# wenzhang-dev/bitcaskDB

Measured on AMD Instinct MI355X. Metric: WAL record decode+CRC GiB/s (device-resident), 4 KiB values, 1/2/4/8 MI355X, higher is better.
Workload: dtype u8; 1 GPU; config B: 1073743514 B WAL segment per GPU, NsSize 20, 100 B keys, 4 KiB values, device-resident decode+CRC+record parse; seg_bytes=1073743514, records=253846, fragments=286402, parallelism=one independent segment per GPU x1

## Files before the change

bitcaskdb_amd/csrc/bcw_decode.hip:

```cpp
#include <hip/hip_runtime.h>

#include <cstdint>

#include "bcw_internal.h"
#include "bcw_parse.h"

namespace bcw {

enum { M_FIRST_BAD = 0,
       M_NE = 1,
       M_NFRAGS = 4, M_DONE_CRC = 5,
       M_T_CRC0 = 10, M_T_FIN = 11,
       M_ABORT = 12,
       M_BAD_CRC = 14,
       M_BAD_TYPE = 15 };

__device__ __forceinline__ uint32_t rotl32(uint32_t x, int r) { return (x << r) | (x >> (32 - r)); }

__device__ __forceinline__ void read_header(const uint8_t* __restrict__ seg, uint64_t seg_len, uint64_t off,
                                            uint32_t& crc, uint32_t& len, uint32_t& type) {
  const uint64_t a = off & ~3ull;
  uint32_t w0, w1, w2;
  if (a + 12 <= seg_len) {
    const uint32_t* q = reinterpret_cast<const uint32_t*>(seg + a);
// ... 412 lines not shown
    const uint64_t be = wg * 64 + 64 < nblocks ? wg * 64 + 64 : nblocks;
    fbase[be] = (uint32_t)(total < 0xffffffffull ? total : 0xffffffffull);
    rbase[be] = (uint32_t)(total_e < 0xffffffffull ? total_e : 0xffffffffull);
    if (wg == nwg - 1) {
      misc[M_NFRAGS] = total;
      misc[M_NE] = total_e;
    }
  }
}

__device__ __forceinline__ uint32_t xor3(uint32_t a, uint32_t b, uint32_t c) {
  return __builtin_amdgcn_bitop3_b32(a, b, c, 0x96);
}
__device__ __forceinline__ uint32_t apply_fwd(const uint32_t* __restrict__ fwd, uint32_t lane, uint32_t x) {
  const uint8_t* b = reinterpret_cast<const uint8_t*>(fwd);
  const uint32_t lane4 = 4u * lane;
  auto at = [&](int i) -> uint32_t {
    const uint32_t sh = 4 * i >= 8 ? (x >> (4 * i - 8)) : (x << (8 - 4 * i));
    return *reinterpret_cast<const uint32_t*>(b + (((sh & 0xf00u) | lane4) + 4096u * (uint32_t)i));
  };
  const uint32_t r0 = at(0), r1 = at(1), r2 = at(2), r3 = at(3), r4 = at(4), r5 = at(5), r6 = at(6), r7 = at(7);
  return xor3(xor3(r0, r1, r2), xor3(r3, r4, r5), r6) ^ r7;
}
__device__ __forceinline__ uint32_t apply_op(const uint32_t* __restrict__ c, uint32_t x) {
  uint32_t r = 0;
#pragma unroll
  for (int i = 0; i < 8; ++i) r ^= c[i * 16 + ((x >> (4 * i)) & 15u)];
  return r;
}

__device__ __forceinline__ uint4 load16_slow(const uint8_t* __restrict__ seg, uint64_t seg_len, int64_t o) {
  uint64_t lo = 0, hi = 0;
#pragma unroll 1
  for (int i = 0; i < 16; ++i) {
    const int64_t q = o + i;
    const uint64_t byte = (q >= 0 && (uint64_t)q < seg_len) ? seg[q] : 0u;
    if (i < 8) lo |= byte << (8 * i); else hi |= byte << (8 * (i - 8));
  }
  return make_uint4((uint32_t)lo, (uint32_t)(lo >> 32), (uint32_t)hi, (uint32_t)(hi >> 32));
}
__device__ __forceinline__ uint4 load16_safe(const uint8_t* __restrict__ seg, uint64_t seg_len, int64_t o) {
  if (o >= 0 && (uint64_t)o + 16 <= seg_len) return *reinterpret_cast<const uint4*>(seg + o);
  return load16_slow(seg, seg_len, o);
}


template <int N>
__device__ __forceinline__ uint32_t reg_byte(const uint32_t (&h)[N], uint32_t pos) {
  uint32_t t[N];
#pragma unroll
  for (int i = 0; i < N; ++i) t[i] = h[i];
  const uint32_t wi = pos >> 2;
  int n = N;
#pragma unroll
  for (int bit = 0; bit < 6; ++bit) {
    if (n <= 1) break;
    const bool hi = (wi >> bit) & 1u;
#pragma unroll
    for (int i = 0; i < (N + 1) / 2; ++i) {
      if (i < (n + 1) / 2) t[i] = (2 * i + 1 < n) ? (hi ? t[2 * i + 1] : t[2 * i]) : t[2 * i];
    }
    n = (n + 1) / 2;
  }
  return (t[0] >> (8u * (pos & 3u))) & 0xffu;
}

constexpr int kHeadWords = 16;
constexpr int kTailWords = 8;

__device__ __attribute__((noinline)) uint32_t walk_byte(const uint8_t* __restrict__ seg, const Frag* __restrict__ frags,
                                                        uint32_t start_off, uint32_t f_first, uint32_t f_last,
                                                        uint64_t pos) {
  uint64_t beg = 0;
  for (uint32_t cf = f_first;; ++cf) {
    const Frag f = frags[cf];
    if (pos < beg + f.len || cf >= f_last)
      return seg[(uint64_t)start_off + (uint64_t)f.blk * kBlock + f.start + (pos - beg)];
    beg += f.len;
  }
}

struct RegReader {
  uint32_t h[kHeadWords];
  uint32_t t[kTailWords];
  uint32_t nhead;
  uint64_t tstart;
  uint64_t tend;
  const uint8_t* seg;
  const Frag* frags;
  uint32_t start_off;
  uint32_t f_first, f_last;
  __device__ __forceinline__ uint32_t operator()(uint64_t pos) {
    if (pos < nhead) return reg_byte(h, (uint32_t)pos);
    if (pos >= tstart && pos < tend) return reg_byte(t, (uint32_t)(pos - tstart));
    return walk_byte(seg, frags, start_off, f_first, f_last, pos);
  }
};

template <int N>
__device__ __forceinline__ void load_words(const uint8_t* __restrict__ seg, uint64_t seg_len, uint64_t base,
                                           uint32_t (&w)[N]) {
  if (base + 4u * N <= seg_len) {
#pragma unroll
    for (int k = 0; k < N / 4; ++k) {
      uint4 v;
      __builtin_memcpy(&v, seg + base + 16 * k, 16);
      w[4 * k + 0] = v.x; w[4 * k + 1] = v.y; w[4 * k + 2] = v.z; w[4 * k + 3] = v.w;
    }
  } else {
#pragma unroll
    for (int k = 0; k < N / 4; ++k) {
      const uint4 v = load16_safe(seg, seg_len, (int64_t)(base + 16 * k));
      w[4 * k + 0] = v.x; w[4 * k + 1] = v.y; w[4 * k + 2] = v.z; w[4 * k + 3] = v.w;
    }
  }
}

struct EmitArgs {
  const uint8_t* seg;
  uint64_t seg_len;
  bcw_decode_params p;
  const Frag* frags;
  const uint32_t* fbase;
  const uint32_t* rbase;
  const uint2* bsum;
  bcw_record_table tab;
  uint64_t* misc;
  uint32_t kb_flags;
  uint64_t* kb_stamps;
};


struct EmitState {
  uint64_t acc;
  int64_t nzb;
  uint32_t nzk, nzs;
  uint64_t rec;
};
__device__ __forceinline__ uint2 emit_prefetch(const EmitArgs& A, uint64_t b0, uint32_t lane) {
  return b0 > lane ? A.bsum[b0 - 1 - lane] : make_uint2(0xffff0000u, kSumHasE);
}

__device__ __forceinline__ EmitState emit_state(const EmitArgs& A, uint64_t b0, uint32_t lane, uint2 s, uint32_t rec) {
  EmitState st{0, -1, 0, 0, rec};
  uint64_t acc = 0;
  for (uint64_t top = b0; top > 0;) {
    if (top != b0) {
      const uint64_t q = top - 1 - lane;
      s = top > lane ? A.bsum[q] : make_uint2(0xffff0000u, kSumHasE);
    }
    const uint64_t he = __ballot((s.y & kSumHasE) != 0u);
    const uint32_t stop = he ? (uint32_t)__builtin_ctzll(he) : 63u;
    const bool contrib = lane <= stop;
    uint32_t ta = contrib ? (s.x & 0xffffu) : 0u;
#pragma unroll
    for (int d = 32; d >= 1; d >>= 1) ta += (uint32_t)__shfl_xor((int)ta, d, 64);
    acc += (uint32_t)__builtin_amdgcn_readfirstlane(ta);
    const uint64_t nzm = __ballot(contrib && (s.x >> 16) != 0xffffu);
    if (nzm) {
      const uint32_t L = 63u - __builtin_clzll(nzm);
      st.nzb = (int64_t)(top - 1 - L);
      st.nzk = (uint32_t)__builtin_amdgcn_readlane((int)(s.x >> 16), L);
      st.nzs = (uint32_t)__builtin_amdgcn_readlane((int)(s.y & 0xffffu), L);
    }
    if (he) break;
    top = top > 64 ? top - 64 : 0;
  }
  st.acc = acc;
  return st;
}

template <bool NOSTORE = false, bool NOPARSE = false, typename Hook>
__device__ __forceinline__ void emit_chunks(const EmitArgs& A, const EmitState& es, uint64_t f0, uint64_t f1,
                                            uint32_t lane, Hook&& hook) {
  if (f0 >= f1) {
    hook();
    return;
  }
  const Frag* __restrict__ frags = A.frags;
  const uint32_t start_off = A.p.start_off;
  uint64_t acc = es.acc, off = 0;
  uint32_t first = 0;
  if (es.nzb >= 0) {
    off = (uint64_t)start_off + (uint64_t)es.nzb * kBlock + es.nzs;
    first = A.fbase[es.nzb] + es.nzk;
  }
  uint64_t rec = es.rec;
  const bool hint = A.p.mode == BCW_MODE_HINT;
  for (uint64_t c0 = f0; c0 < f1; c0 += 64) {
    const uint64_t g = c0 + lane;
    const bool valid = g < f1;
    const uint4 fr = reinterpret_cast<const uint4*>(frags)[valid ? g : f1 - 1];
    if (c0 == f0) hook();
    Frag f;
    __builtin_memcpy(&f, &fr, sizeof f);
    if (!valid) f = Frag{};
    const uint32_t len = valid ? f.len : 0u;
    const uint64_t D = (uint64_t)start_off + (uint64_t)f.blk * kBlock + f.start;
    const bool isE = valid && (f.type == BCW_RECORD_FULL || f.type == BCW_RECORD_LAST);
    const uint64_t E = __ballot(isE);
    const uint64_t NZ = __ballot(valid && len > 0);
    const uint32_t S = wave_add_scan(len, lane);
    const uint64_t below = (lane == 0) ? 0ull : (~0ull >> (64 - lane));
    const uint64_t pm = E & below;
    const int prev = pm ? 63 - __builtin_clzll(pm) : -1;
    const uint32_t S_prev = __shfl(S, prev < 0 ? 0 : prev, 64);
    const uint64_t between = (uint64_t)(S - len) - (prev < 0 ? 0u : S_prev);
    const uint64_t acc_before = (prev < 0 ? acc : 0ull) + between;
    const uint64_t range = prev < 0 ? below : (below & ~(~0ull >> (63 - prev)));
    const uint64_t nzr = NZ & range;
    const int fnz = nzr ? __builtin_ctzll(nzr) : 0;
    const uint64_t D_fnz = __shfl(D, fnz, 64);
    const uint64_t V = __ballot(valid);
    const int last_valid = V ? 63 - __builtin_clzll(V) : -1;
    const uint32_t S_tot = __shfl(S, last_valid < 0 ? 0 : last_valid, 64);
    const int lastE = E ? 63 - __builtin_clzll(E) : -1;
    uint64_t acc2, off2;
    uint32_t first2;
    {
      const uint32_t S_lastE = __shfl(S, lastE < 0 ? 0 : lastE, 64);
      const uint64_t after = lastE < 0 ? V : (V & ~(~0ull >> (63 - lastE)));
      const uint64_t nza = NZ & after;
      const int fa = nza ? __builtin_ctzll(nza) : 0;
      const uint64_t D_fa = __shfl(D, fa, 64);
      if (lastE >= 0) {
        acc2 = (uint64_t)(S_tot - S_lastE);
        off2 = D_fa;
        first2 = (uint32_t)(c0 + fa);
      } else {
        acc2 = acc + S_tot;
        if (acc > 0 || !nza) { off2 = off; first2 = first; }
        else { off2 = D_fa; first2 = (uint32_t)(c0 + fa); }
      }
    }
    uint64_t foff;
    uint32_t ffrag;
    if (acc_before == 0) { foff = D; ffrag = (uint32_t)g; }
    else if (prev < 0 && acc > 0) { foff = off; ffrag = first; }
    else { foff = D_fnz; ffrag = (uint32_t)(c0 + fnz); }
    const bool full = f.type == BCW_RECORD_FULL;
    const uint32_t src = full ? (uint32_t)g : ffrag;
    const bool src_here = src >= c0 && src < c0 + 64;
    const uint32_t sw0 = (uint32_t)__shfl((int)f.blk, src_here ? (int)(src - c0) : (int)lane, 64);
    const uint32_t sw1 = (uint32_t)__shfl((int)((uint32_t)f.start | ((uint32_t)f.len << 16)),
                                          src_here ? (int)(src - c0) : (int)lane, 64);
    const bool nx_here = src + 1u >= c0 && src + 1u < c0 + 64;
    const uint32_t sx0 = (uint32_t)__shfl((int)f.blk, nx_here ? (int)(src + 1u - c0) : (int)lane, 64);
    const uint32_t sx1 = (uint32_t)__shfl((int)((uint32_t)f.start | ((uint32_t)f.len << 16)),
                                          nx_here ? (int)(src + 1u - c0) : (int)lane, 64);
    if (isE) {
      const uint64_t size = full ? (uint64_t)len : acc_before + len;
      const uint64_t r = rec + __builtin_popcountll(E & below);
      Frag fs = f;
      if (!full) {
        if (src_here) { fs.blk = sw0; fs.start = (uint16_t)sw1; fs.len = (uint16_t)(sw1 >> 16); }
        else fs = frags[src];
      }
      RegReader rd;
      const uint64_t a0 = (uint64_t)start_off + (uint64_t)fs.blk * kBlock + fs.start;
      uint64_t want = size < 64u ? size : 64u;
      if (want > fs.len) want = fs.len;
      rd.nhead = (uint32_t)want;
      load_words(A.seg, A.seg_len, a0, rd.h);
      rd.tstart = rd.tend = ~0ull;
      if (hint) {
        uint64_t nt = size < 32u ? size : 32u;
        if (nt > len) nt = len;
        rd.tstart = size - nt;
        load_words(A.seg, A.seg_len, D + len - nt, rd.t);
      } else if (want < (size < 64u ? size : 64u)) {
        Frag f2;
        if (nx_here) { f2.blk = sx0; f2.start = (uint16_t)sx1; f2.len = (uint16_t)(sx1 >> 16); }
        else f2 = frags[src + 1u];
        load_words(A.seg, A.seg_len, (uint64_t)start_off + (uint64_t)f2.blk * kBlock + f2.start, rd.t);
        uint64_t n2 = f2.len < 32u ? f2.len : 32u;
        if (n2 > size - want) n2 = size - want;
        rd.tstart = want;
        rd.tend = want + n2;
      } else {
#pragma unroll
        for (int k = 0; k < kTailWords; ++k) rd.t[k] = 0;
      }
      rd.seg = A.seg; rd.frags = frags; rd.start_off = start_off;
      rd.f_first = src; rd.f_last = (uint32_t)g;
      uint8_t status, hdr, flags, etag_off;
      uint64_t key_len, val_len, meta_len, expire, aux0, aux1;
      if (NOPARSE) {
        status = 0; hdr = (uint8_t)rd.h[0]; flags = (uint8_t)rd.h[5]; etag_off = 0;
        key_len = rd.h[6] ^ rd.h[9]; val_len = rd.h[7] ^ rd.h[12]; meta_len = rd.h[8] ^ rd.h[15]; expire = rd.h[10];
        aux0 = rd.t[0]; aux1 = rd.t[1];
      } else {
        parse_record(A.p, rd, size, status, hdr, flags, etag_off, key_len, val_len, meta_len, expire, aux0, aux1);
      }
      const bcw_record_table& tab = A.tab;
      if (NOSTORE) {
        if (status == 0xeeu) tab.foff[r] = foff ^ size ^ expire ^ aux0 ^ aux1 ^ key_len ^ val_len ^ meta_len ^ hdr ^ flags ^ etag_off;
      } else if (r < tab.capacity) {
        tab.foff[r] = foff;
        tab.size[r] = size;
        tab.expire[r] = expire;
        if (tab.aux0) tab.aux0[r] = aux0;
        if (tab.aux1) tab.aux1[r] = aux1;
        tab.key_len[r] = (uint32_t)key_len;
        tab.val_len[r] = (uint32_t)val_len;
        tab.meta_len[r] = (uint32_t)meta_len;
        tab.first_frag[r] = src;
        tab.emit_frag[r] = (uint32_t)g;
        tab.hdr_size[r] = hdr;
        tab.flags[r] = flags;
        tab.etag_off[r] = etag_off;
        tab.status[r] = status;
      }
      if (status != BCW_ST_OK) atomicMin((unsigned long long*)&A.misc[M_FIRST_BAD], (unsigned long long)r);
    }
    rec += __builtin_popcountll(E);
    acc = acc2;
    off = off2;
    first = first2;
  }
}

struct ItemMeta {
  uint64_t bb;
  uint2 s;
  uint32_t f0, f1, rec;
};
__device__ __forceinline__ uint32_t ld_const(const uint32_t* p, uint64_t i) {
  return ((const __attribute__((address_space(4))) uint32_t*)p)[i];
}
__device__ __forceinline__ ItemMeta item_meta(const EmitArgs& A, uint64_t it, uint64_t bpw, uint64_t cb0, uint64_t cb1,
                                              uint32_t lane) {
  ItemMeta m;
  m.bb = cb0 + it * bpw < cb1 ? cb0 + it * bpw : cb1 - 1;
  const uint64_t be = m.bb + bpw < cb1 ? m.bb + bpw : cb1;
  m.s = emit_prefetch(A, m.bb, lane);
  m.f0 = ld_const(A.fbase, m.bb);
  m.f1 = ld_const(A.fbase, be);
  m.rec = ld_const(A.rbase, m.bb);
  return m;
}

__device__ __forceinline__ void finalize(const EmitArgs& A, uint64_t nblocks, uint64_t frag_cap, uint32_t tail_panic, uint64_t gen,
                         bcw_decode_result* __restrict__ res, uint32_t lane) {
  uint64_t* misc = A.misc;
  const uint64_t bad_crc = __hip_atomic_load(&misc[M_BAD_CRC], __ATOMIC_RELAXED, __HIP_MEMORY_SCOPE_AGENT);
  const uint64_t bad_type = __hip_atomic_load(&misc[M_BAD_TYPE], __ATOMIC_RELAXED, __HIP_MEMORY_SCOPE_AGENT);
  const uint64_t fb = __hip_atomic_load(&misc[M_FIRST_BAD], __ATOMIC_RELAXED, __HIP_MEMORY_SCOPE_AGENT);
  const uint64_t nfr = __hip_atomic_load(&misc[M_NFRAGS], __ATOMIC_RELAXED, __HIP_MEMORY_SCOPE_AGENT);
  const uint64_t abort_site = __hip_atomic_load(&misc[M_ABORT], __ATOMIC_RELAXED, __HIP_MEMORY_SCOPE_AGENT);
  const uint64_t err = bad_crc < bad_type ? bad_crc : bad_type;
  uint64_t lim = err < frag_cap ? err : frag_cap;
  uint64_t nrec = __hip_atomic_load(&misc[M_NE], __ATOMIC_RELAXED, __HIP_MEMORY_SCOPE_AGENT);
  if (lim < nfr && abort_site == 0ull) {
    uint64_t lo = 0, hi = nblocks;
    while (hi - lo > 1) {
      const uint64_t step = (hi - lo + 63) / 64;
      const uint64_t q = lo + (uint64_t)lane * step;
      const bool le = q < hi && A.fbase[q] <= lim;
      const uint64_t m = __ballot(le);
      const uint32_t L = m ? 63u - __builtin_clzll(m) : 0u;
      lo = lo + (uint64_t)L * step;
      hi = lo + step < hi ? lo + step : hi;
    }
    uint64_t cnt = 0;
    for (uint64_t c0 = A.fbase[lo]; c0 < lim; c0 += 64) {
      const uint64_t g = c0 + lane;
      const uint32_t ty = g < lim ? A.frags[g].type : 0u;
      cnt += (uint64_t)__builtin_popcountll(__ballot(ty == BCW_RECORD_FULL || ty == BCW_RECORD_LAST));
    }
    nrec = (uint64_t)A.rbase[lo] + cnt;
  }
  if (lane != 0) return;
  bcw_decode_result r{};
  r.n_records = nrec;
  r.n_records_total = nrec;
  r.err_frag = err;
  r.err_class = err == ~0ull ? BCW_ERR_NONE : (bad_crc <= bad_type ? BCW_ERR_CRC : BCW_ERR_TYPE);
  r.n_frags = err != ~0ull ? err + 1 : nfr;
  if (r.err_class == BCW_ERR_NONE && tail_panic) r.err_class = BCW_ERR_PANIC;
  if (abort_site != 0ull) {
    r.err_class = BCW_ERR_INTERNAL;
    r.err_frag = abort_site;
    r.n_records = r.n_records_total = 0;
    nrec = 0;
  }
  r.err_file_off = 0;
  if (err != ~0ull && err < frag_cap && abort_site == 0ull) {
    const Frag f = A.frags[err];
    r.err_file_off = (uint64_t)A.p.start_off + (uint64_t)f.blk * kBlock + f.start - kHdr;
  }
  r.first_bad_record = fb < nrec ? (int32_t)(fb < 0x7fffffffull ? fb : 0x7fffffffull) : -1;
  r.n_blocks = nblocks;
  r.retry_frag_capacity = (nfr > frag_cap && abort_site == 0ull) ? nfr : 0;
  r.generation = gen;
  *res = r;
  if (abort_site != 0ull) misc[M_NFRAGS] = 0;
  misc[M_DONE_CRC] = 0;
  misc[M_BAD_CRC] = ~0ull;
  misc[M_FIRST_BAD] = ~0ull;
  misc[M_BAD_TYPE] = ~0ull;
  misc[M_ABORT] = 0;
}

struct StreamFrag {
  int64_t gs, ge;
  uint32_t J;
};

struct SliceLane2 {
  uint32_t base;
  uint32_t sel[4];
};
__device__ __forceinline__ SliceLane2 slice_lane2(uint32_t lane) {
  SliceLane2 s;
  const uint32_t g = (lane >> 3) & 3u, copy = lane & 7u;
  s.base = 0;
#pragma unroll
  for (uint32_t k = 0; k < 4; ++k) {
    const uint32_t slot = (k + g) & 3u;
    s.base |= (slot * 32u + copy * 4u) << (8u * k);
    s.sel[k] = 0x0c0c0000u | ((4u + slot) << 8) | k;
  }
  return s;
}
template <bool SH>
__device__ __forceinline__ uint32_t slice4_step2(const uint8_t* __restrict__ tb, const SliceLane2& sl, uint32_t x,
                                                 uint32_t next) {
  constexpr uint32_t o = SH ? 128u : 0u;
  const uint32_t a0 = *reinterpret_cast<const uint32_t*>(tb + __builtin_amdgcn_perm(x, sl.base, sl.sel[0]) + o);
  const uint32_t a1 = *reinterpret_cast<const uint32_t*>(tb + __builtin_amdgcn_perm(x, sl.base, sl.sel[1]) + o);
  const uint32_t a2 = *reinterpret_cast<const uint32_t*>(tb + __builtin_amdgcn_perm(x, sl.base, sl.sel[2]) + o);
  const uint32_t a3 = *reinterpret_cast<const uint32_t*>(tb + __builtin_amdgcn_perm(x, sl.base, sl.sel[3]) + o);
  return xor3(xor3(a0, a1, a2), a3, next);
}
template <bool CAP>
__device__ __forceinline__ uint32_t chain_piece2(const uint8_t* __restrict__ tb, const SliceLane2& sl, uint32_t seed,
                                                 const uint32_t (&w)[kSPW], uint32_t K = 0, uint32_t* cap = nullptr) {
  uint32_t x = seed ^ w[0];
  uint32_t st[kSPW - 1];
#pragma unroll
  for (int q = 0; q < kSPW - 1; ++q) {
    x = slice4_step2<false>(tb, sl, x, w[q + 1]);
    if (CAP) st[q] = x ^ w[q + 1];
  }
  if (CAP) *cap = K == 1u ? st[0] : (K == 2u ? st[1] : st[2]);
  return slice4_step2<true>(tb, sl, x, 0u);
}

__device__ __forceinline__ uint64_t c_safe_bound(uint64_t seg_len) { return (seg_len + 4u + kSChunk - 1u) / kSChunk; }

__device__ __forceinline__ uint4 lds_entry(const uint32_t* __restrict__ tab, uint32_t idx) {
  return *reinterpret_cast<const uint4*>(tab + 4u * idx);
}
__device__ __forceinline__ void mask_gap(uint32_t (&x)[kSPW], const uint32_t (&w)[kSPW], int32_t pb, uint32_t J,
                                         uint32_t lane, const uint32_t* __restrict__ lds) {
  const uint32_t g = min((uint32_t)(pb - (int32_t)(kSPiece * lane) + 6), (uint32_t)(kS2GapN - 1));
  const uint4 S = lds_entry(lds + kS2Gap, g);
  x[0] = __builtin_amdgcn_perm(J, w[0], S.x);
  x[1] = __builtin_amdgcn_perm(J, w[1], S.y);
  x[2] = __builtin_amdgcn_perm(J, w[2], S.z);
  x[3] = __builtin_amdgcn_perm(J, w[3], S.w);
}
__device__ __forceinline__ void mask_chunk(uint32_t (&x)[kSPW], const uint32_t (&w)[kSPW], int32_t pa, int32_t pb,
                                           int32_t pc, uint32_t J, uint32_t lane, const uint32_t* __restrict__ lds) {
  const int32_t q = (int32_t)(kSPiece * lane);
  const uint4 A = lds_entry(lds + kS2Ge, (uint32_t)min(max(pa - q, 0), kS2GeN - 1));
// ... 177 lines not shown
};
__device__ __forceinline__ XBalIn xbal_load(const XBal* __restrict__ xb, uint32_t lane) {
  const uint32_t y = lane & 7u;
  XBalIn v;
  v.t = __hip_atomic_load(&xb->t[y], __ATOMIC_RELAXED, __HIP_MEMORY_SCOPE_AGENT);
  v.n = __hip_atomic_load(&xb->n[y], __ATOMIC_RELAXED, __HIP_MEMORY_SCOPE_AGENT);
  v.w = xb->w[y];
  v.on = xb->on;
  return v;
}
__device__ __forceinline__ void xbal_update(XBal* __restrict__ xb, uint32_t lane, const XBalIn& in) {
  const uint32_t y = lane & 7u;
  const uint64_t t = in.t, n = in.n;
  const float Ty = n && t ? (float)t / (float)n : 0.0f;
  const bool all = __ballot(lane < 8u && Ty > 0.0f) == 0xffull && in.on != 0u;
  float sT = lane < 8u ? Ty : 0.0f;
#pragma unroll
  for (int d = 32; d >= 1; d >>= 1) sT += __shfl_xor(sT, d, 64);
  if (lane < 8u) {
    if (all) {
      const float wy = (float)in.w * (1.0f + 0.5f * ((sT / 8.0f) / Ty - 1.0f));
      const float d = fminf(fmaxf(rintf((wy - 65536.0f) / 256.0f), -51.0f), 64.0f);
      xb->w[y] = (uint32_t)(65536 + 256 * (int32_t)d);
    }
    xb->t[y] = 0;
    xb->n[y] = 0;
  }
}

template <int ABL = 0>
__global__ __launch_bounds__(kCrcThreads) void k_crc(const uint8_t* __restrict__ seg, uint64_t seg_len,
                                                     uint32_t start_off, uint64_t nblocks,
                                                     const uint32_t* __restrict__ fbase, uint8_t* __restrict__ fok,
                                                     const uint4* __restrict__ srec,
                                                     uint64_t frag_cap, Tables tabs, EmitArgs ea,
                                                     uint32_t tail_panic, uint64_t gen,
                                                     bcw_decode_result* __restrict__ res,
                                                     uint64_t* __restrict__ misc, uint64_t cb0, uint64_t cb1,
                                                     uint32_t nwg_total, const uint32_t* __restrict__ wstart,
                                                     XBal* __restrict__ xb) {
  __shared__ __attribute__((aligned(16))) uint32_t lds[kS2Image];
  __shared__ CrcTail s_tail;
  __shared__ uint32_t s_wdone;
  __shared__ uint32_t s_eq;
  __shared__ __attribute__((aligned(16))) uint32_t s_rem[kCrcWaves];
  __shared__ uint32_t s_sdone;
  __shared__ unsigned long long s_tsum;
  __shared__ uint64_t s_t0;
  const uint32_t tid = threadIdx.x;
  const uint32_t lane = tid & 63u;
  const uint32_t wave = __builtin_amdgcn_readfirstlane(tid >> 6);
  if (tid < (uint32_t)kCrcWaves) s_rem[tid] = 0;
  if (ea.kb_stamps && lane == 0) {
    uint64_t* q = ea.kb_stamps + 8 * ((uint64_t)blockIdx.x * kCrcWaves + wave);
    q[4] = wall_clock64();
    q[5] = __builtin_amdgcn_s_memtime();
    q[7] = ((uint64_t)__builtin_amdgcn_s_getreg(20 | (31 << 11)) << 32) | __builtin_amdgcn_s_getreg(4 | (31 << 11));
  }
  if (tid == 0) {
    s_wdone = 0;
    s_eq = 0;
    s_sdone = 0;
    s_tsum = 0;
    s_t0 = wall_clock64();
    s_tail = CrcTail{ea, res, misc, nblocks, frag_cap, gen, cb0, cb1, tail_panic, nwg_total};
  }
  {
    const uint4* src4 = reinterpret_cast<const uint4*>(tabs.lds_image2);
    uint4* dst4 = reinterpret_cast<uint4*>(lds);
    constexpr uint32_t kLop4 = kS2SliceOff / 4, kKop4 = kS2KopOff / 4, kEnd4 = kS2Image / 4;
    constexpr uint32_t kN4 = kLop4 + (kEnd4 - kKop4);
    constexpr int kPer = (int)((kN4 + kCrcThreads - 1) / kCrcThreads);
    static_assert(kS2Slice == 256 * 64 && kCrcThreads * 2 == 256 * 8, "slice rows: 256 x 8 distinct dwords");
    auto at = [](uint32_t i) { return i < kLop4 ? i : i - kLop4 + kKop4; };
    uint4 v[kPer];
#pragma unroll
    for (int k2 = 0; k2 < kPer; ++k2) {
      const uint32_t i = tid + k2 * kCrcThreads;
      v[k2] = i < kN4 ? src4[at(i)] : make_uint4(0, 0, 0, 0);
    }
    const uint32_t* src1 = tabs.lds_image2 + kS2SliceOff;
    uint32_t sv[2];
#pragma unroll
    for (int k2 = 0; k2 < 2; ++k2) {
      const uint32_t t = tid + k2 * kCrcThreads;
      sv[k2] = src1[(t >> 3) * 64u + (t & 7u) * 8u];
    }
#pragma unroll
    for (int k2 = 0; k2 < kPer; ++k2) {
      const uint32_t i = tid + k2 * kCrcThreads;
      if (i < kN4) dst4[at(i)] = v[k2];
    }
#pragma unroll
    for (int k2 = 0; k2 < 2; ++k2) {
      const uint32_t t = tid + k2 * kCrcThreads;
      uint4* d = reinterpret_cast<uint4*>(lds + kS2SliceOff + (t >> 3) * 64u + (t & 7u) * 8u);
      d[0] = make_uint4(sv[k2], sv[k2], sv[k2], sv[k2]);
      d[1] = make_uint4(sv[k2], sv[k2], sv[k2], sv[k2]);
    }
  }
  __syncthreads();
  const uint64_t gw = (uint64_t)blockIdx.x * kCrcWaves + wave;
  const uint64_t f0 = wstart[gw];
  uint64_t f1 = wstart[gw + 1];
  if (f1 > frag_cap) f1 = frag_cap;
  if (f0 > f1) f1 = f0;
  const bool aborted = __builtin_amdgcn_readfirstlane(
                           (uint32_t)__hip_atomic_load(&misc[M_ABORT], __ATOMIC_RELAXED, __HIP_MEMORY_SCOPE_AGENT)) != 0u;
  if (aborted) f1 = f0;
  if (blockIdx.x == 0 && tid == 0) misc[M_T_CRC0] = wall_clock64();
  const uint32_t nfr = f1 > f0 ? (uint32_t)(f1 - f0) : 0u;
  uint64_t n_items = 0;
  auto emit_items = [&](uint64_t max_items) {
    asm volatile("" ::: "memory");
    CrcTail T;
    {
      static_assert(sizeof(CrcTail) % 4 == 0, "CrcTail words");
      const uint32_t* src = reinterpret_cast<const uint32_t*>(&s_tail);
      uint32_t* dst = reinterpret_cast<uint32_t*>(&T);
#pragma unroll
      for (int k = 0; k < (int)(sizeof(CrcTail) / 4); ++k) dst[k] = __builtin_amdgcn_readfirstlane(src[k]);
    }
    const EmitArgs& A = T.ea;
    if ((ABL & 8) || (A.kb_flags & 1u) ||
        __builtin_amdgcn_readfirstlane(
            (uint32_t)__hip_atomic_load(&T.misc[M_ABORT], __ATOMIC_RELAXED, __HIP_MEMORY_SCOPE_AGENT)) != 0u)
      return;
    const uint64_t cb0t = T.cb0, cb1t = T.cb1, fcap = T.frag_cap;
    const uint32_t cnt = (uint32_t)(cb1t - cb0t), G = gridDim.x, wg = blockIdx.x;
    const uint64_t fc0 = A.fbase[cb0t], fc1 = A.fbase[cb1t];
    const uint32_t nf_all = (uint32_t)(fc1 > fc0 ? (fc1 - fc0 < fcap ? fc1 - fc0 : fcap) : 0);
    uint32_t bpw = nf_all ? (64u * cnt) / nf_all : cnt;
    if (bpw < 1u) bpw = 1u;
    bpw = __builtin_amdgcn_readfirstlane(bpw);
    const uint32_t cq = cnt / G, cr = cnt % G;
    const uint32_t B0 = cq * wg + (cr * wg) / G, B1 = cq * (wg + 1u) + (cr * (wg + 1u)) / G;
    const uint64_t i0 = __builtin_amdgcn_readfirstlane((B0 + bpw - 1u) / bpw),
                   nitems = __builtin_amdgcn_readfirstlane((B1 + bpw - 1u) / bpw);
    auto deq = [&]() -> uint64_t {
      uint32_t j = 0;
      if (lane == 0) j = atomicAdd(&s_eq, 1u);
      j = __builtin_amdgcn_readfirstlane(j);
      return i0 + j;
    };
    uint64_t taken = 0;
    uint64_t it = deq();
    ItemMeta m = item_meta(A, it, bpw, cb0t, cb1t, lane);
    while (it < nitems) {
      ++taken;
      const EmitState es = emit_state(A, m.bb, lane, m.s, m.rec);
      const uint64_t mf1 = m.f1 < fcap ? m.f1 : fcap;
      uint64_t nx = ~0ull;
      ItemMeta mn = m;
      emit_chunks<(ABL & 4096) != 0, (ABL & 131072) != 0>(A, es, m.f0, mf1, lane, [&]() {
        if (taken < max_items) {
          nx = deq();
          mn = item_meta(A, nx, bpw, cb0t, cb1t, lane);
        }
      });
      it = nx;
      m = mn;
    }
    n_items += taken;
  };
  if (ABL & 64) emit_items(~0ull);
  if (ABL & 16384) {
    for (uint32_t q = 0; q < 4u; ++q) {
      const uint32_t a = nfr * q / 4u, b = nfr * (q + 1u) / 4u;
      stream_verify<(ABL & 8388608) != 0>(seg, seg_len, fok, srec, f0 + a, b - a, lds, lane, misc, s_rem,
                                          (wave & 3u) * 4u + (wave >> 2),
                                          reinterpret_cast<const uint8_t*>(tabs.lds_image2));
    }
  } else if (!(ABL & 32768))
    stream_verify<(ABL & 8388608) != 0>(seg, seg_len, fok, srec, f0, nfr, lds, lane, misc, s_rem,
                                        (wave & 3u) * 4u + (wave >> 2),
                                        reinterpret_cast<const uint8_t*>(tabs.lds_image2));
  __builtin_amdgcn_s_setprio(0);
  if (lane == 0) {
    atomicAdd(&s_tsum, (unsigned long long)(wall_clock64() - s_t0));
    if (atomicAdd(&s_sdone, 1u) == kCrcWaves - 1u) {
      const uint32_t c = blockIdx.x & 7u;
      __hip_atomic_fetch_add(&xb->t[c], (uint64_t)s_tsum, __ATOMIC_RELAXED, __HIP_MEMORY_SCOPE_AGENT);
      __hip_atomic_fetch_add(&xb->n[c], (uint64_t)kCrcWaves, __ATOMIC_RELAXED, __HIP_MEMORY_SCOPE_AGENT);
    }
  }
  if (ea.kb_stamps && lane == 0) {
    uint64_t* q = ea.kb_stamps + 8 * ((uint64_t)blockIdx.x * kCrcWaves + wave);
    q[0] = wall_clock64();
    q[3] = nfr;
  }
  if (!(ABL & 64)) emit_items(~0ull);
  asm volatile("" ::: "memory");
  CrcTail T;
  {
    const uint32_t* src = reinterpret_cast<const uint32_t*>(&s_tail);
    uint32_t* dst = reinterpret_cast<uint32_t*>(&T);
#pragma unroll
    for (int k = 0; k < (int)(sizeof(CrcTail) / 4); ++k) dst[k] = __builtin_amdgcn_readfirstlane(src[k]);
  }
  const EmitArgs& A = T.ea;
  if (A.kb_stamps && lane == 0) {
    uint64_t* q = A.kb_stamps + 8 * ((uint64_t)__builtin_amdgcn_workgroup_id_x() * kCrcWaves + wave);
    q[1] = wall_clock64(); q[2] = n_items;
    q[6] = __builtin_amdgcn_s_memtime();
  }
  asm volatile("s_waitcnt vmcnt(0)" ::: "memory");
  __builtin_amdgcn_fence(__ATOMIC_RELEASE, "workgroup");
  uint32_t order = 0;
  if (lane == 0) order = atomicAdd(&s_wdone, 1u);
  order = __builtin_amdgcn_readlane(order, 0);
  if (order != kCrcWaves - 1) return;
  __builtin_amdgcn_fence(__ATOMIC_ACQUIRE, "workgroup");
  uint64_t gorder = 0;
  if (lane == 0)
    gorder = __hip_atomic_fetch_add(&T.misc[M_DONE_CRC], 1ull, __ATOMIC_RELAXED, __HIP_MEMORY_SCOPE_AGENT);
  gorder = (uint64_t)__shfl((long long)gorder, 0, 64);
  if (gorder != T.nwg_total - 1u) return;
  if (lane == 0) T.misc[M_T_FIN] = wall_clock64();
  const XBalIn xin = xbal_load(xb, lane);
  finalize(A, T.nblocks, T.frag_cap, T.tail_panic, T.gen, T.res, lane);
  xbal_update(xb, lane, xin);
}

__global__ void k_export_frags(const Frag* __restrict__ frags, const uint8_t* __restrict__ fok,
                               const uint64_t* __restrict__ misc, uint64_t cap,
                               uint32_t start_off, bcw_frag_table out, const uint32_t* __restrict__ initc) {
  const uint64_t g = blockIdx.x * (uint64_t)blockDim.x + threadIdx.x;
  const uint64_t n = misc[M_NFRAGS];
  if (g >= n || g >= cap || g >= out.capacity) return;
  const Frag f = frags[g];
  out.data_off[g] = (uint64_t)start_off + (uint64_t)f.blk * kBlock + f.start;
  out.len[g] = f.len;
  const uint32_t u = ~(f.chk ^ initc[f.len]);
  out.stored_crc[g] = ((u >> 15) | (u << 17)) + 0xa282ead8u;
  out.type[g] = f.type;
  out.crc_ok[g] = fok[g];
}



hipError_t launch_decode(const uint8_t* d_seg, const bcw_decode_params& p, const bcw_record_table& t,
                         bcw_decode_result* d_result, const Tables& tabs, Scratch& s, uint64_t nblocks,
                         uint64_t gen, hipStream_t stream, int num_cus, Prof* prof) {
  Prof dummy;
  Prof& pr = prof ? *prof : dummy;
  hipEvent_t ev = nullptr;
  const uint64_t tail = (p.seg_len - p.start_off) % kBlock;
  const uint32_t tail_panic = (tail > 0 && tail < kHdr) ? 1u : 0u;
  const uint32_t nb_grid = (uint32_t)(((nblocks + 63) / 64 + 7) / 8 * 8);
  const EmitArgs ea{d_seg, p.seg_len, p, s.frags, s.fbase, s.rbase, s.bsum, t, s.misc, 0u, nullptr};
  pr.begin(K_CHASE, stream, ev);
  k_chase<0><<<nb_grid, 64, 0, stream>>>(d_seg, p.seg_len, p.start_off, nblocks, s.fbase, s.rbase, s.bsum, s.frags,
                                        s.srec, s.frag_cap, s.lb, s.lbe, s.misc, s.epoch, tabs.initc, s.chase_direct,
                                        s.test_abort_wg, s.wstart, (uint32_t)num_cus * kCrcWaves, s.xbal, s.xbal_on);
  s.test_abort_wg = 0;
  pr.end(K_CHASE, stream, ev);
  if ((++s.epoch & 0xffffffull) == 0) {
    (void)hipMemsetAsync(s.lb, 0, s.nlb * sizeof(uint64_t), stream);
    (void)hipMemsetAsync(s.lbe, 0, s.nlb * sizeof(uint64_t), stream);
    s.epoch = 1;
  }
  pr.begin(K_CRC, stream, ev);
  k_crc<0><<<(uint32_t)num_cus, kCrcThreads, 0, stream>>>(d_seg, p.seg_len, p.start_off, nblocks, s.fbase, s.fok,
                                                         s.srec, s.frag_cap, tabs, ea,
                                                         tail_panic, gen, d_result, s.misc, 0ull, nblocks,
                                                         (uint32_t)num_cus, s.wstart, s.xbal);
  pr.end(K_CRC, stream, ev);
  return hipGetLastError();
}

hipError_t launch_export_frags(const Scratch& s, const bcw_frag_table& out, uint32_t start_off, hipStream_t stream,
                               uint64_t n, const uint32_t* initc) {
  if (n == 0) return hipSuccess;
  k_export_frags<<<(uint32_t)((n + 255) / 256), 256, 0, stream>>>(s.frags, s.fok, s.misc, s.frag_cap, start_off, out,
                                                                    initc);
  return hipGetLastError();
}

}
```

bitcaskdb_amd/csrc/bcw_parse.h:

```cpp
#pragma once
#include <hip/hip_runtime.h>

#include <cstdint>

#include "bcw.h"

namespace bcw {

template <typename RD>
__device__ __forceinline__ uint64_t uvarint(RD& rd, uint64_t pos, uint64_t len, uint32_t& used) {
  uint64_t x = 0;
  uint32_t s = 0;
#pragma unroll 1
  for (uint32_t i = 0; pos + i < len; ++i) {
    if (i == 10) { used = 0; return 0; }
    const uint32_t b = rd(pos + i);
    if (b < 0x80u) {
      if (i == 9 && b > 1u) { used = 0; return 0; }
      used = i + 1;
      return x | ((uint64_t)b << s);
    }
    x |= (uint64_t)(b & 0x7fu) << s;
    s += 7;
  }
  used = 0;
  return 0;
}

template <typename RD>
__device__ __forceinline__ void parse_record(const bcw_decode_params& p, RD& rd, uint64_t len, uint8_t& status,
                                             uint8_t& hdr, uint8_t& flags, uint8_t& etag_off, uint64_t& key_len,
                                             uint64_t& val_len, uint64_t& meta_len, uint64_t& expire, uint64_t& aux0,
                                             uint64_t& aux1) {
  uint32_t used;
  status = BCW_ST_OK;
  hdr = flags = etag_off = 0;
  key_len = val_len = meta_len = expire = aux0 = aux1 = 0;
  if (p.mode == BCW_MODE_RECORD) {
    const uint64_t min_hdr = 1ull + p.ns_size + 1ull + 3ull;
    if (len < min_hdr) { status = BCW_ST_INVALID; return; }
    const uint64_t header = rd(0);
    uint64_t o = 1 + p.ns_size;
    const uint32_t flag = rd(o);
    ++o;
    key_len = uvarint(rd, o, len, used); o += used;
    val_len = uvarint(rd, o, len, used); o += used;
    meta_len = uvarint(rd, o, len, used); o += used;
    const uint64_t etag_len = (flag & 1u) ? 0 : p.etag_size;
    uint64_t expire_size = 0;
    hdr = (uint8_t)header; flags = (uint8_t)flag; etag_off = (uint8_t)o;
    if ((flag & 2u) == 0) {
      if (o + etag_len > len) { status = BCW_ST_PANIC; return; }
      expire = uvarint(rd, o + etag_len, len, used);
      expire_size = used;
      expire += p.base_time;
    }
    const int64_t cur_hdr = (int64_t)o + (int64_t)etag_len + (int64_t)expire_size;
    const int64_t cur_total = cur_hdr + (int64_t)(key_len + val_len + meta_len);
    if ((uint64_t)cur_hdr != header || cur_total != (int64_t)len) { status = BCW_ST_INVALID; return; }
    const uint64_t s1 = key_len + val_len;
    const uint64_t s2 = s1 + meta_len;
    const bool wrapped = (s1 < key_len) || (s2 < s1);
    if ((int64_t)key_len < 0 || (int64_t)val_len < 0 || (int64_t)meta_len < 0 || wrapped) status = BCW_ST_PANIC;
    else if (key_len > 0xffffffffull || val_len > 0xffffffffull || meta_len > 0xffffffffull || len > 0xffffffffull)
      status = BCW_ST_UNSUPPORTED;
  } else {
    if (len < (uint64_t)p.ns_size + 5ull) { status = BCW_ST_INVALID; return; }
    int64_t o = p.ns_size;
    key_len = uvarint(rd, (uint64_t)o, len, used);
    o += used;
    const int64_t key_off = o;
    o = (int64_t)((uint64_t)o + key_len);
    hdr = (uint8_t)key_off;
    if (o < 0 || o > (int64_t)len) { status = BCW_ST_PANIC; return; }
    expire = uvarint(rd, (uint64_t)o, len, used); o += used;
    aux0 = uvarint(rd, (uint64_t)o, len, used); o += used;
    aux1 = uvarint(rd, (uint64_t)o, len, used); o += used;
    if (o != (int64_t)len) status = BCW_ST_INVALID;
    else if ((int64_t)key_len < 0) status = BCW_ST_PANIC;
  }
}

}
```

Measured before the change: 4997 GiB/s.

## Add windowed branchless record-header parse with fallback to byte reader

Measured after the change: 4996 GiB/s. No clear change (-0.0%).

```diff
diff --git a/bitcaskdb_amd/csrc/bcw_decode.hip b/bitcaskdb_amd/csrc/bcw_decode.hip
--- a/bitcaskdb_amd/csrc/bcw_decode.hip
+++ b/bitcaskdb_amd/csrc/bcw_decode.hip
@@ -588,10 +588,8 @@
     const uint64_t he = __ballot((s.y & kSumHasE) != 0u);
     const uint32_t stop = he ? (uint32_t)__builtin_ctzll(he) : 63u;
     const bool contrib = lane <= stop;
-    uint32_t ta = contrib ? (s.x & 0xffffu) : 0u;
-#pragma unroll
-    for (int d = 32; d >= 1; d >>= 1) ta += (uint32_t)__shfl_xor((int)ta, d, 64);
-    acc += (uint32_t)__builtin_amdgcn_readfirstlane(ta);
+    const uint32_t ta = contrib ? (s.x & 0xffffu) : 0u;
+    acc += (uint32_t)__builtin_amdgcn_readlane(wave_add_scan(ta, lane), 63);
     const uint64_t nzm = __ballot(contrib && (s.x >> 16) != 0xffffu);
     if (nzm) {
       const uint32_t L = 63u - __builtin_clzll(nzm);
@@ -606,7 +604,89 @@
   return st;
 }
 
-template <bool NOSTORE = false, bool NOPARSE = false, typename Hook>
+template <bool NOSTORE, bool NOPARSE, bool READERPARSE, typename Next, typename Last>
+__device__ __forceinline__ void emit_one(const EmitArgs& A, uint64_t r, uint64_t foff, uint64_t size, uint32_t src,
+                                         uint32_t g, const Frag& fs, Next&& next, Last&& last) {
+  const Frag* __restrict__ frags = A.frags;
+  const uint32_t start_off = A.p.start_off;
+  const bool hint = A.p.mode == BCW_MODE_HINT;
+  const uint32_t winB = (A.p.ns_size < 0xffffu ? A.p.ns_size : 0xffffu) + 1u;
+  const uint64_t a0 = (uint64_t)start_off + (uint64_t)fs.blk * kBlock + fs.start;
+  uint8_t status, hdr, flags, etag_off;
+  uint64_t key_len, val_len, meta_len, expire, aux0, aux1;
+  bool parsed = false;
+  if (!NOPARSE && !READERPARSE && !hint) {
+    uint32_t w[4];
+    const uint32_t header = A.seg[a0 < A.seg_len ? a0 : A.seg_len - 1u];
+    load_words(A.seg, A.seg_len, a0 + winB, w);
+    const uint64_t held = size < fs.len ? size : fs.len;
+    const uint32_t n = held > winB ? (uint32_t)(held - winB < 16u ? held - winB : 16u) : 0u;
+    parsed = parse_record_win(
+        A.p, size, header, w[0], w[1], w[2], w[3], n,
+        [&](uint64_t pos, uint32_t (&x)[4], uint32_t& n2) {
+          n2 = held > pos ? (uint32_t)(held - pos < 16u ? held - pos : 16u) : 0u;
+          if (n2) load_words(A.seg, A.seg_len, a0 + pos, x);
+          else x[0] = x[1] = x[2] = x[3] = 0u;
+        },
+        status, hdr, flags, etag_off, key_len, val_len, meta_len, expire, aux0, aux1);
+  }
+  if (!parsed) {
+    RegReader rd;
+    uint64_t want = size < 64u ? size : 64u;
+    if (want > fs.len) want = fs.len;
+    rd.nhead = (uint32_t)want;
+    load_words(A.seg, A.seg_len, a0, rd.h);
+    rd.tstart = rd.tend = ~0ull;
+    if (hint) {
+      const Frag fl = last();
+      uint64_t nt = size < 32u ? size : 32u;
+      if (nt > fl.len) nt = fl.len;
+      rd.tstart = size - nt;
+      load_words(A.seg, A.seg_len, (uint64_t)start_off + (uint64_t)fl.blk * kBlock + fl.start + fl.len - nt, rd.t);
+    } else if (want < (size < 64u ? size : 64u)) {
+      const Frag f2 = next();
+      load_words(A.seg, A.seg_len, (uint64_t)start_off + (uint64_t)f2.blk * kBlock + f2.start, rd.t);
+      uint64_t n2 = f2.len < 32u ? f2.len : 32u;
+      if (n2 > size - want) n2 = size - want;
+      rd.tstart = want;
+      rd.tend = want + n2;
+    } else {
+#pragma unroll
+      for (int k = 0; k < kTailWords; ++k) rd.t[k] = 0;
+    }
+    rd.seg = A.seg; rd.frags = frags; rd.start_off = start_off;
+    rd.f_first = src; rd.f_last = g;
+    if (NOPARSE) {
+      status = 0; hdr = (uint8_t)rd.h[0]; flags = (uint8_t)rd.h[5]; etag_off = 0;
+      key_len = rd.h[6] ^ rd.h[9]; val_len = rd.h[7] ^ rd.h[12]; meta_len = rd.h[8] ^ rd.h[15]; expire = rd.h[10];
+      aux0 = rd.t[0]; aux1 = rd.t[1];
+    } else {
+      parse_record(A.p, rd, size, status, hdr, flags, etag_off, key_len, val_len, meta_len, expire, aux0, aux1);
+    }
+  }
+  const bcw_record_table& tab = A.tab;
+  if (NOSTORE) {
+    if (status == 0xeeu) tab.foff[r] = foff ^ size ^ expire ^ aux0 ^ aux1 ^ key_len ^ val_len ^ meta_len ^ hdr ^ flags ^ etag_off;
+  } else if (r < tab.capacity) {
+    tab.foff[r] = foff;
+    tab.size[r] = size;
+    tab.expire[r] = expire;
+    if (tab.aux0) tab.aux0[r] = aux0;
+    if (tab.aux1) tab.aux1[r] = aux1;
+    tab.key_len[r] = (uint32_t)key_len;
+    tab.val_len[r] = (uint32_t)val_len;
+    tab.meta_len[r] = (uint32_t)meta_len;
+    tab.first_frag[r] = src;
+    tab.emit_frag[r] = g;
+    tab.hdr_size[r] = hdr;
+    tab.flags[r] = flags;
+    tab.etag_off[r] = etag_off;
+    tab.status[r] = status;
+  }
+  if (status != BCW_ST_OK) atomicMin((unsigned long long*)&A.misc[M_FIRST_BAD], (unsigned long long)r);
+}
+
+template <bool NOSTORE = false, bool NOPARSE = false, bool READERPARSE = false, typename Hook>
 __device__ __forceinline__ void emit_chunks(const EmitArgs& A, const EmitState& es, uint64_t f0, uint64_t f1,
                                             uint32_t lane, Hook&& hook) {
   if (f0 >= f1) {
@@ -622,7 +702,6 @@
     first = A.fbase[es.nzb] + es.nzk;
   }
   uint64_t rec = es.rec;
-  const bool hint = A.p.mode == BCW_MODE_HINT;
   for (uint64_t c0 = f0; c0 < f1; c0 += 64) {
     const uint64_t g = c0 + lane;
     const bool valid = g < f1;
@@ -680,10 +759,6 @@
     const uint32_t sw0 = (uint32_t)__shfl((int)f.blk, src_here ? (int)(src - c0) : (int)lane, 64);
     const uint32_t sw1 = (uint32_t)__shfl((int)((uint32_t)f.start | ((uint32_t)f.len << 16)),
                                           src_here ? (int)(src - c0) : (int)lane, 64);
-    const bool nx_here = src + 1u >= c0 && src + 1u < c0 + 64;
-    const uint32_t sx0 = (uint32_t)__shfl((int)f.blk, nx_here ? (int)(src + 1u - c0) : (int)lane, 64);
-    const uint32_t sx1 = (uint32_t)__shfl((int)((uint32_t)f.start | ((uint32_t)f.len << 16)),
-                                          nx_here ? (int)(src + 1u - c0) : (int)lane, 64);
     if (isE) {
       const uint64_t size = full ? (uint64_t)len : acc_before + len;
       const uint64_t r = rec + __builtin_popcountll(E & below);
@@ -692,62 +767,8 @@
         if (src_here) { fs.blk = sw0; fs.start = (uint16_t)sw1; fs.len = (uint16_t)(sw1 >> 16); }
         else fs = frags[src];
       }
-      RegReader rd;
-      const uint64_t a0 = (uint64_t)start_off + (uint64_t)fs.blk * kBlock + fs.start;
-      uint64_t want = size < 64u ? size : 64u;
-      if (want > fs.len) want = fs.len;
-      rd.nhead = (uint32_t)want;
-      load_words(A.seg, A.seg_len, a0, rd.h);
-      rd.tstart = rd.tend = ~0ull;
-      if (hint) {
-        uint64_t nt = size < 32u ? size : 32u;
-        if (nt > len) nt = len;
-        rd.tstart = size - nt;
-        load_words(A.seg, A.seg_len, D + len - nt, rd.t);
-      } else if (want < (size < 64u ? size : 64u)) {
-        Frag f2;
-        if (nx_here) { f2.blk = sx0; f2.start = (uint16_t)sx1; f2.len = (uint16_t)(sx1 >> 16); }
-        else f2 = frags[src + 1u];
-        load_words(A.seg, A.seg_len, (uint64_t)start_off + (uint64_t)f2.blk * kBlock + f2.start, rd.t);
-        uint64_t n2 = f2.len < 32u ? f2.len : 32u;
-        if (n2 > size - want) n2 = size - want;
-        rd.tstart = want;
-        rd.tend = want + n2;
-      } else {
-#pragma unroll
-        for (int k = 0; k < kTailWords; ++k) rd.t[k] = 0;
-      }
-      rd.seg = A.seg; rd.frags = frags; rd.start_off = start_off;
-      rd.f_first = src; rd.f_last = (uint32_t)g;
-      uint8_t status, hdr, flags, etag_off;
-      uint64_t key_len, val_len, meta_len, expire, aux0, aux1;
-      if (NOPARSE) {
-        status = 0; hdr = (uint8_t)rd.h[0]; flags = (uint8_t)rd.h[5]; etag_off = 0;
-        key_len = rd.h[6] ^ rd.h[9]; val_len = rd.h[7] ^ rd.h[12]; meta_len = rd.h[8] ^ rd.h[15]; expire = rd.h[10];
-        aux0 = rd.t[0]; aux1 = rd.t[1];
-      } else {
-        parse_record(A.p, rd, size, status, hdr, flags, etag_off, key_len, val_len, meta_len, expire, aux0, aux1);
-      }
-      const bcw_record_table& tab = A.tab;
-      if (NOSTORE) {
-        if (status == 0xeeu) tab.foff[r] = foff ^ size ^ expire ^ aux0 ^ aux1 ^ key_len ^ val_len ^ meta_len ^ hdr ^ flags ^ etag_off;
-      } else if (r < tab.capacity) {
-        tab.foff[r] = foff;
-        tab.size[r] = size;
-        tab.expire[r] = expire;
-        if (tab.aux0) tab.aux0[r] = aux0;
-        if (tab.aux1) tab.aux1[r] = aux1;
-        tab.key_len[r] = (uint32_t)key_len;
-        tab.val_len[r] = (uint32_t)val_len;
-        tab.meta_len[r] = (uint32_t)meta_len;
-        tab.first_frag[r] = src;
-        tab.emit_frag[r] = (uint32_t)g;
-        tab.hdr_size[r] = hdr;
-        tab.flags[r] = flags;
-        tab.etag_off[r] = etag_off;
-        tab.status[r] = status;
-      }
-      if (status != BCW_ST_OK) atomicMin((unsigned long long*)&A.misc[M_FIRST_BAD], (unsigned long long)r);
+      emit_one<NOSTORE, NOPARSE, READERPARSE>(A, r, foff, size, src, (uint32_t)g, fs,
+                                              [&]() -> Frag { return frags[src + 1u]; }, [&]() -> Frag { return f; });
     }
     rec += __builtin_popcountll(E);
     acc = acc2;
@@ -1231,7 +1252,7 @@
       const uint64_t mf1 = m.f1 < fcap ? m.f1 : fcap;
       uint64_t nx = ~0ull;
       ItemMeta mn = m;
-      emit_chunks<(ABL & 4096) != 0, (ABL & 131072) != 0>(A, es, m.f0, mf1, lane, [&]() {
+      emit_chunks<(ABL & 4096) != 0, (ABL & 131072) != 0, (ABL & 262144) != 0>(A, es, m.f0, mf1, lane, [&]() {
         if (taken < max_items) {
           nx = deq();
           mn = item_meta(A, nx, bpw, cb0t, cb1t, lane);
diff --git a/bitcaskdb_amd/csrc/bcw_parse.h b/bitcaskdb_amd/csrc/bcw_parse.h
--- a/bitcaskdb_amd/csrc/bcw_parse.h
+++ b/bitcaskdb_amd/csrc/bcw_parse.h
@@ -8,7 +8,7 @@
 namespace bcw {
 
 template <typename RD>
-__device__ __forceinline__ uint64_t uvarint(RD& rd, uint64_t pos, uint64_t len, uint32_t& used) {
+__host__ __device__ __forceinline__ uint64_t uvarint(RD& rd, uint64_t pos, uint64_t len, uint32_t& used) {
   uint64_t x = 0;
   uint32_t s = 0;
 #pragma unroll 1
@@ -28,7 +28,7 @@
 }
 
 template <typename RD>
-__device__ __forceinline__ void parse_record(const bcw_decode_params& p, RD& rd, uint64_t len, uint8_t& status,
+__host__ __device__ __forceinline__ void parse_record(const bcw_decode_params& p, RD& rd, uint64_t len, uint8_t& status,
                                              uint8_t& hdr, uint8_t& flags, uint8_t& etag_off, uint64_t& key_len,
                                              uint64_t& val_len, uint64_t& meta_len, uint64_t& expire, uint64_t& aux0,
                                              uint64_t& aux1) {
@@ -81,4 +81,83 @@
   }
 }
 
+struct WinRec {
+  uint32_t flag, key_len, val_len, meta_len;
+  uint32_t o;
+  uint32_t expire;
+  uint32_t expire_size;
+};
+
+__host__ __device__ __forceinline__ uint32_t win_bytes4(uint64_t lo, uint64_t hi, uint32_t s) {
+  const uint64_t a = s < 8u ? lo : (s < 16u ? hi : 0ull), c = s < 8u ? hi : 0ull;
+  const uint32_t b = 8u * (s & 7u);
+  return (uint32_t)(b ? (a >> b) | (c << (64u - b)) : a);
 }
+
+__host__ __device__ __forceinline__ bool win_varint(uint64_t lo, uint64_t hi, uint32_t n, uint32_t& s, uint32_t& v,
+                                                    uint32_t& used) {
+  const uint32_t x = win_bytes4(lo, hi, s);
+  const uint32_t stop = ~x & 0x80808080u;
+  const uint32_t nb = stop ? ((uint32_t)__builtin_ctz(stop) >> 3) + 1u : 5u;
+  const uint32_t y = x & (0xffffffffu >> (32u - 8u * (nb < 4u ? nb : 4u)));
+  v = (y & 0x7fu) | ((y >> 1) & 0x3f80u) | ((y >> 2) & 0x1fc000u) | ((y >> 3) & 0xfe00000u);
+  used = nb;
+  const bool ok = (nb <= 4u) & (s + nb <= n);
+  s += nb;
+  return ok;
+}
+
+__host__ __device__ __forceinline__ bool win_decode(uint32_t w0, uint32_t w1, uint32_t w2, uint32_t w3, uint32_t n,
+                                                    uint32_t etag_size, WinRec& r, bool& expire_ok) {
+  const uint64_t lo = (uint64_t)w0 | (uint64_t)w1 << 32, hi = (uint64_t)w2 | (uint64_t)w3 << 32;
+  if (n > 16u) n = 16u;
+  r.flag = w0 & 0xffu;
+  uint32_t s = 1, used;
+  bool ok = n >= 1u;
+  ok &= win_varint(lo, hi, n, s, r.key_len, used);
+  ok &= win_varint(lo, hi, n, s, r.val_len, used);
+  ok &= win_varint(lo, hi, n, s, r.meta_len, used);
+  r.o = s;
+  const bool has_expire = (r.flag & 2u) == 0u;
+  const uint32_t etag_len = (r.flag & 1u) ? 0u : (etag_size < 16u ? etag_size : 16u);
+  uint32_t e = s + etag_len, ev, eu;
+  const bool eok = win_varint(lo, hi, n, e, ev, eu);
+  expire_ok = !has_expire | eok;
+  r.expire = has_expire ? ev : 0u;
+  r.expire_size = has_expire ? eu : 0u;
+  return ok;
+}
+
+template <typename More>
+__host__ __device__ __forceinline__ bool parse_record_win(const bcw_decode_params& p, uint64_t len, uint32_t header,
+                                                          uint32_t w0, uint32_t w1, uint32_t w2, uint32_t w3,
+                                                          uint32_t n, More&& more, uint8_t& status, uint8_t& hdr,
+                                                          uint8_t& flags, uint8_t& etag_off, uint64_t& key_len,
+                                                          uint64_t& val_len, uint64_t& meta_len, uint64_t& expire,
+                                                          uint64_t& aux0, uint64_t& aux1) {
+  WinRec w;
+  bool expire_ok;
+  const uint64_t min_hdr = 1ull + p.ns_size + 1ull + 3ull;
+  if (len < min_hdr || !win_decode(w0, w1, w2, w3, n, p.etag_size, w, expire_ok)) return false;
+  const uint64_t o = 1ull + p.ns_size + w.o;
+  const uint64_t etag_len = (w.flag & 1u) ? 0 : p.etag_size;
+  if (!expire_ok) {
+    uint32_t x[4], n2 = 0, s = 0;
+    more(o + etag_len, x, n2);
+    if (n2 > 16u) n2 = 16u;
+    if (!win_varint((uint64_t)x[0] | (uint64_t)x[1] << 32, (uint64_t)x[2] | (uint64_t)x[3] << 32, n2, s, w.expire,
+                    w.expire_size))
+      return false;
+  }
+  status = BCW_ST_OK;
+  aux0 = aux1 = 0;
+  key_len = w.key_len; val_len = w.val_len; meta_len = w.meta_len;
+  hdr = (uint8_t)header; flags = (uint8_t)w.flag; etag_off = (uint8_t)o;
+  expire = (w.flag & 2u) == 0 ? (uint64_t)w.expire + p.base_time : 0ull;
+  const int64_t cur_hdr = (int64_t)o + (int64_t)etag_len + (int64_t)w.expire_size;
+  const int64_t cur_total = cur_hdr + (int64_t)(key_len + val_len + meta_len);
+  if ((uint64_t)cur_hdr != (uint64_t)(header & 0xffu) || cur_total != (int64_t)len) status = BCW_ST_INVALID;
+  return true;
+}
+
+}
```
